# guenthermi/postgres-word2vec

Measured on AMD Instinct MI355X. Metric: batched IVFADC kNN queries/sec (k=5) + recall@5, 3Mx300d, higher is better.
Workload: dtype f32; 1 GPU; IVFADC batch (ivfadc_batch_search generalised to nprobe), 3000000x300d, C=1000, m=12, K=1024, nprobe=10, k=5, batch=1024 queries per GPU, replicated index, queries sharded by rank; N=3000000, d=300, C=1000, m=12, K=1024, nprobe=10, k=5, batch_per_gpu=1024, parallelism=dp1, world_size=1, backend=none (single GPU), batches_in_flight=4

## Files before the change

postgres-word2vec_amd/csrc/core.hip:

```cpp
#include "internal.h"

static thread_local char g_err[512] = "";

int fail(int code, const char* fmt, ...) {
  va_list ap;
  va_start(ap, fmt);
  vsnprintf(g_err, sizeof(g_err), fmt, ap);
  va_end(ap);
  return code;
}

extern "C" const char* freddy_gpu_last_error(void) { return g_err; }

#include "registry.h"

void backend_handles(int delta, int device) { freddy::registry::handles(delta, device); }
int backends_other(bool searching, int device) { return freddy::registry::others(searching, device); }
void backend_busy(int delta) { freddy::registry::busy(delta); }
void choose_hw_queues(int device) {
  static std::once_flag once;
  std::call_once(once, [device] {
    const char* policy = getenv("FREDDY_GPU_HWQ_POLICY");
    const bool alone = backends_other(false, device) == 0;
    const char* q = (policy && *policy && strcmp(policy, "registry") != 0) ? policy : (alone ? "6" : "2");
    setenv("GPU_MAX_HW_QUEUES", q, 0);
  });
}

int64_t env_int(const char* name, int64_t dflt) {
  const char* e = getenv(name);
  return (e && *e) ? (int64_t)strtoll(e, nullptr, 10) : dflt;
}
Tuning read_tuning() {
  Tuning t;
  t.fused = (int)env_int("FREDDY_GPU_FUSED", t.fused);
  t.scan_kernel = (int)env_int("FREDDY_GPU_FUSED_KERNEL", t.scan_kernel);
  t.reserve_cus = (int)env_int("FREDDY_GPU_RESERVE_CUS", 0);
  t.scan_share = (int)std::max<int64_t>(0, env_int("FREDDY_GPU_SCAN_SHARE", t.scan_share));
  t.pipeline_batch = (int)std::max<int64_t>(16, env_int("FREDDY_GPU_PIPELINE_BATCH", t.pipeline_batch));
  t.pipeline_lanes = (int)std::min<int64_t>(4, std::max<int64_t>(1, env_int("FREDDY_GPU_PIPELINE_LANES", t.pipeline_lanes)));
  t.pq_fused = (int)env_int("FREDDY_GPU_PQ_FUSED", t.pq_fused);
  t.one_launch = (int)env_int("FREDDY_GPU_ONE_LAUNCH", t.one_launch);
  t.coarse_approx = (int)env_int("FREDDY_GPU_COARSE_APPROX", 1);
  t.sparse_items = (int)env_int("FREDDY_GPU_SPARSE_ITEMS", t.sparse_items);
  t.exact_filter = (int)env_int("FREDDY_GPU_EXACT_FILTER", t.exact_filter);
  t.codes_u8 = (int)env_int("FREDDY_GPU_CODES_U8", t.codes_u8);
  t.running_bound = (int)env_int("FREDDY_GPU_RUNNING_BOUND", t.running_bound);
  t.lut_budget_mb = std::max<int64_t>(1, env_int("FREDDY_GPU_LUT_BUDGET_MB", t.lut_budget_mb));
  t.lane0_own = (int)env_int("FREDDY_GPU_LANE0_OWN", t.lane0_own);
  t.coarse_pieces = (int)env_int("FREDDY_GPU_COARSE_PIECES", t.coarse_pieces);
#ifdef FREDDY_LAB
  t.scan_prof = getenv("FREDDY_GPU_FUSED_PROF") != nullptr;
#endif
  return t;
}

Workspace* workspace_for(freddy_gpu_index* ix, hipStream_t s) {
  std::lock_guard<std::mutex> lock(ix->mu);
  Workspace* w = nullptr;
  for (Workspace& c : ix->ws)
    if (c.used && c.owner == s) { w = &c; break; }
  if (!w)
    for (Workspace& c : ix->ws)
      if (!c.used) { c.used = true; c.owner = s; w = &c; break; }
  if (!w) {
    w = &ix->ws[0];
    for (Workspace& c : ix->ws)
      if (c.last_use < w->last_use) w = &c;
    (void)hipDeviceSynchronize();
    w->owner = s;
  }
  w->last_use = ++ix->ws_clock;
  ix->last_ws = w;
  return w;
}

void free_index(freddy_gpu_index* ix) {
  if (!ix) return;
  if (ix->registered) { ix->registered = false; backend_handles(-1, ix->device); }
  for (freddy_gpu_index* r : ix->replicas) free_index(r);
  ix->replicas.clear();
  (void)hipSetDevice(ix->device);
  (void)hipDeviceSynchronize();
// ... 122 lines not shown
  if (!ix || !name) return fail(FREDDY_E_ARG, "NULL argument");
  if (!ix->replicas.empty()) {
    std::vector<freddy_gpu_index*> reps;
    reps.swap(ix->replicas);
    int rc = freddy_gpu_set_option(ix, name, value);
    reps.swap(ix->replicas);
    if (rc) return rc;
    for (freddy_gpu_index* r : ix->replicas)
      if ((rc = freddy_gpu_set_option(r, name, value))) { ix->poisoned = true; return rc; }
    return FREDDY_OK;
  }
  Tuning& t = ix->tune;
  const std::string n(name);
  if (n == "fused") t.fused = (int)value;
  else if (n == "fused_kernel") t.scan_kernel = (int)value;
  else if (n == "reserve_cus") t.reserve_cus = (int)value;
  else if (n == "scan_share") t.scan_share = (int)std::max<int64_t>(0, value);
  else if (n == "join_host_traversal") ix->join.host_traversal = value != 0;
  else if (n == "join_libm_margin_ppm") ix->join.libm_margin = (float)value * 1e-6f;
  else if (n == "sparse_items") t.sparse_items = std::max(-16, std::min(16, (int)value));
  else if (n == "pipeline_batch") t.pipeline_batch = (int)std::max<int64_t>(16, value);
  else if (n == "pipeline_lanes") t.pipeline_lanes = (int)std::min<int64_t>(FREDDY_LANES, std::max<int64_t>(1, value));
  else if (n == "pq_fused") t.pq_fused = (int)value;
  else if (n == "one_launch") t.one_launch = (int)value;
  else if (n == "coarse_approx") t.coarse_approx = (int)value;
  else if (n == "check_brackets") t.check_brackets = (int)value;
  else if (n == "lut_budget_mb") t.lut_budget_mb = std::max<int64_t>(1, value);
  else if (n == "exact_filter") t.exact_filter = (int)value;
  else if (n == "exact_join_tile") t.exact_join_tile = (int)value;
  else if (n == "analogy_pass") t.analogy_pass = (int)std::max<int64_t>(0, std::min<int64_t>(value, 1 << 30));
  else if (n == "codes_u8") t.codes_u8 = (int)value;
  else if (n == "running_bound") t.running_bound = (int)value;
  else if (n == "coarse_pieces") t.coarse_pieces = (int)value;
#ifdef FREDDY_LAB
  else if (n == "fused_prof") t.scan_prof = (int)value;
  else if (n == "scan_fence") t.scan_fence = (int)value;
#endif
  else return fail(FREDDY_E_ARG, "unknown option '%s'", name);
  return FREDDY_OK;
}

int check_search_args(const freddy_gpu_index* ix, int kind, const void* q, int Q, int k, const void* oi,
                             const void* od) {
  if (!ix) return fail(FREDDY_E_ARG, "NULL index");
  if (ix->kind != kind) return fail(FREDDY_E_KIND, "index handle has the wrong kind for this call");
  if (ix->poisoned) return fail(FREDDY_E_HIP, "this handle's devices hold different tables (an append / codebook update failed part-way): unpin it and pin again");
  if (Q < 0 || k <= 0) return fail(FREDDY_E_ARG, "Q must be >= 0 and k > 0");
  if (Q > 0 && (!q || !oi || !od)) return fail(FREDDY_E_ARG, "NULL buffer");
  if (k > 4096) return fail(FREDDY_E_LIMIT, "k=%d exceeds this build's limit of 4096", k);
  return 0;
}

extern "C" int freddy_gpu_host_alloc(void** out, size_t bytes) {
  choose_hw_queues(-1);
  if (!out) return fail(FREDDY_E_ARG, "NULL argument");
  *out = nullptr;
  if (hipHostMalloc(out, bytes ? bytes : 1, hipHostMallocDefault) != hipSuccess) { *out = nullptr; return fail(FREDDY_E_NOMEM, "pinned host allocation of %zu bytes failed", bytes); }
  return FREDDY_OK;
}
extern "C" int freddy_gpu_host_free(void* p) {
  if (p) HIP_TRY(hipHostFree(p));
  return FREDDY_OK;
}

extern "C" int freddy_gpu_replica_count(const freddy_gpu_index_t* ix) { return ix ? 1 + (int)ix->replicas.size() : 0; }
extern "C" int freddy_gpu_abi_version(void) { return FREDDY_GPU_ABI_VERSION; }
// ... 1 lines not shown
```

postgres-word2vec_amd/csrc/fused5.h:

```cpp
#pragma once
#include <hip/hip_runtime.h>
#include <stdint.h>

#include "refine.h"
#include "coarse.h"
#include "scan_tail5.h"

namespace freddy {

static constexpr int SCAN5_G = 16;

__host__ __device__ __forceinline__ constexpr int filt5_bias(int p, int m) { return FILT5_VMAX + (p < 32768 - FILT5_VMAX * m ? 1 : 0); }
__device__ __forceinline__ uint32_t lane_byte4() {
  uint32_t x;
  asm volatile("v_mbcnt_lo_u32_b32 %0, -1, 0\n\tv_mbcnt_hi_u32_b32 %0, -1, %0\n\tv_lshlrev_b32 %0, 2, %0" : "=v"(x));
  return x;
}
typedef short s2v __attribute__((ext_vector_type(2)));
__device__ __forceinline__ uint32_t pk_add_i16(uint32_t x, uint32_t y) {
  return __builtin_bit_cast(uint32_t, __builtin_bit_cast(s2v, x) + __builtin_bit_cast(s2v, y));
}

template <int S, int QT>
__device__ __forceinline__ void query_codebook5_body(const float* __restrict__ queries, const float* __restrict__ cbT,
// ... 91 lines not shown
                                                             const float* __restrict__ cmax, float* __restrict__ qn,
                                                             float* __restrict__ qscale, uint32_t* __restrict__ qc,
                                                             int Q, int d, int m, int K, uint32_t* __restrict__ qc8) {
  __shared__ __attribute__((aligned(16))) unsigned char smem[query_codebook5_lds<S, QT>()];
  query_codebook5_body<S, QT>(queries, cbT, cmax, qn, qscale, qc, Q, d, m, K, blockIdx.x, blockIdx.y, smem, qc8);
}

struct CoarseTableArgs {
  const float* queries;
  const float* coarseF; const float* cn2; float* dist; float* qn2; int Q, Cpad, d, dp; ZeroArgs z; int coarse_gx, coarse_gy;
  const float* cbT; const float* cmax; float* qn; float* qscale; uint32_t* qc; int m, K;
  float* tmin; int C;
  const ch8v* coarseH; int ec;
  uint32_t* qc8;
};
template <int S, int QT, bool H16 = false>
__global__ __launch_bounds__(256) void coarse_table5_kernel(CoarseTableArgs a) {
  extern __shared__ __attribute__((aligned(16))) unsigned char smem[];
  const int n_coarse = a.coarse_gx * a.coarse_gy;
  const int b = blockIdx.x;
  if (b < n_coarse) {
    if constexpr (H16)
      coarse_approx16_body(a.queries, a.coarseH, a.ec, a.cn2, a.dist, a.qn2, a.Q, a.Cpad, a.d, a.z, b % a.coarse_gx, b / a.coarse_gx,
                           a.coarse_gx, a.coarse_gy, smem, a.tmin, a.C);
    else
    coarse_approx_body(a.queries, a.coarseF, a.cn2, a.dist, a.qn2, a.Q, a.Cpad, a.d, a.dp, a.z, b % a.coarse_gx, b / a.coarse_gx,
                       a.coarse_gx, a.coarse_gy, smem, a.tmin, a.C);
  } else {
    const int t = b - n_coarse;
    query_codebook5_body<S, QT>(a.queries, a.cbT, a.cmax, a.qn, a.qscale, a.qc, a.Q, a.d, a.m, a.K, t % a.m, t / a.m, smem, a.qc8);
  }
}

template <int M>
__global__ __launch_bounds__(256) void entry_record5_kernel(RecordArgs a) {
  const int lane = threadIdx.x & 63;
  const int e = blockIdx.x * 4 + (threadIdx.x >> 6);
  if (e >= a.n_groups[0]) return;
  const int cell = a.group_cell[e], first = a.group_first[e], gc = a.group_cnt[e];
  const int cnt = gc & 0xff, chunk = gc >> 8;
  int32_t* rec = a.records + (size_t)e * REC_DW;
  if (lane == 0) {
    const int b0 = a.blk_off[cell] + chunk * FUSED_UNIT_BLOCKS;
    int nb = a.blk_off[cell + 1] - b0;
    if (nb > FUSED_UNIT_BLOCKS) nb = FUSED_UNIT_BLOCKS;
    int rows = a.list_off[cell + 1] - a.list_off[cell] - chunk * (FUSED_UNIT_BLOCKS * 64);
    if (rows > FUSED_UNIT_BLOCKS * 64) rows = FUSED_UNIT_BLOCKS * 64;
    rec[0] = cell; rec[1] = cnt; rec[2] = chunk; rec[3] = b0; rec[4] = nb; rec[5] = rows;
  }
  if (lane < 16) {
    const int it = lane < cnt ? a.sorted_item[first + lane] : -1;
    const int q = a.item_query[it >= 0 ? it : a.sorted_item[first]];
    const float sc = a.qscale[q];
    ItemBounds ib = item_bounds(0.0f, 0.0f, a.sentinel);
    if (it >= 0) ib = item_bounds(a.item_dist[it], filter_width5<M>(a.qn + (size_t)q * M, a.pmax, sc), a.sentinel);
    rec[8 + lane] = it;
    rec[24 + lane] = q;
    rec[40 + lane] = (int32_t)__float_as_uint(ib.off);
    rec[56 + lane] = (int32_t)__float_as_uint(ib.e);
    rec[72 + lane] = (int32_t)__float_as_uint(ib.shift);
    rec[88 + lane] = (int32_t)ib.lo_bits;
    rec[104 + lane] = (int32_t)ib.hi_bits;
    rec[128 + lane] = (int32_t)__float_as_uint((it >= 0 && sc < 1e30f) ? sc : 0.0f);
    const float A = it >= 0 ? a.item_dist[it] : -1.0f;
    const bool fin = it >= 0 && ib.e < 1e30f && A >= 0.0f && A < 1e30f;
    rec[144 + lane] = (int32_t)__float_as_uint(fin ? A * (1.0f + 2e-5f) : __uint_as_float(0x7f800000u));
    rec[160 + lane] = (int32_t)__float_as_uint(fin ? A * (1.0f - 2e-5f) : 0.0f);
  }
}

template <int M, bool FULLK, bool CAND, bool PROF = false, bool U8 = false>
__global__ __launch_bounds__(SPEC2_T) void ivf_filter5_kernel(FilterArgs a) {
  static_assert(!(U8 && FULLK), "one byte per code: K <= 256");
  constexpr int G = SCAN5_G, RMAX = FUSED_RMAX, NG = SPEC2_NG;
  constexpr int NP = M / 2;
  constexpr int ROWB = G * 2;
  constexpr int HROWB = 16;
  static_assert(M == 12 && G == 16 && SPEC2_NB == 8, "layout");
  typedef uint32_t u2 __attribute__((ext_vector_type(2)));
  typedef uint32_t u4 __attribute__((ext_vector_type(4)));
  extern __shared__ __attribute__((aligned(16))) unsigned char smem[];
  unsigned char* slab = smem;
  uint32_t* colmin = reinterpret_cast<uint32_t*>(smem + a.desc_offset);
  uint32_t* thr_s = colmin + 16 * 64;
  int32_t* dsc = reinterpret_cast<int32_t*>(smem + a.desc_offset + 4096 + 64);
  int32_t* gidq = dsc + 2 * REC_DW;
  float* rt_s = reinterpret_cast<float*>(gidq + 4);

  const int tid = threadIdx.x, lane = tid & 63;
  const int wave = __builtin_amdgcn_readfirstlane(tid >> 6);
  const bool builder = wave < SPEC2_NB;
  const int K = FULLK ? 1024 : a.K;
  const uint32_t HALFB = (uint32_t)K * HROWB;
  const uint32_t POSB = 2u * HALFB;
  const uint32_t BUFB = 2u * POSB;
  const int n_work = a.n_groups[0];

  int cur = 0, ei = 0;
  if (tid == 0) { gidq[0] = (int)blockIdx.x; gidq[1] = (int)gridDim.x + atomicAdd(a.work_counter, 1); }
  if (tid < REC_DW) dsc[tid] = a.records[(size_t)blockIdx.x * REC_DW + tid];
  for (int i = tid; i < 16 * 64; i += SPEC2_T) colmin[i] = 0xffffffffu;
// ... 283 lines not shown
```

postgres-word2vec_amd/csrc/internal.h:

```cpp
#pragma once
#include "../../include/freddy_gpu.h"

#include <hip/hip_runtime.h>

#include <algorithm>
#include <atomic>
#include <thread>
#include <cmath>
#include <cstdarg>
#include <cstdio>
#include <cstdlib>
#include <cstring>
#include <limits>
#include <chrono>
#include <map>
#include <mutex>
#include <string>
#include <type_traits>
#include <vector>

#include "join_index.h"
#include "pinned.h"

using namespace freddy;

int fail(int code, const char* fmt, ...) __attribute__((format(printf, 2, 3)));

#define HIP_TRY(expr)                                                                       \
  do {                                                                                      \
    hipError_t e_ = (expr);                                                                 \
    if (e_ != hipSuccess)                                                                   \
      return fail(FREDDY_E_HIP, "%s failed: %s (%s:%d)", #expr, hipGetErrorString(e_),      \
                  __FILE__, __LINE__);                                                      \
  } while (0)

enum { KIND_PQ = 1, KIND_IVF = 2, KIND_IVPQ = 3, KIND_VEC = 4 };

struct Tuning {
  int scan_share = 0;
  int reserve_cus = 0;
  int pipeline_batch = 2048;
  int pipeline_lanes = 4;
  int lane0_own = 0;
  int coarse_pieces = 1;
  int64_t lut_budget_mb = 8192;
  int fused = -1;
  int scan_kernel = 5;
  int coarse_approx = 1;
  int one_launch = 1;
  int pq_fused = -1;
  int sparse_items = 2;
  int running_bound = 1;
  int codes_u8 = 1;
  int exact_filter = -1;
  int exact_join_tile = 0;
  int analogy_pass = 0;
  int check_brackets = 0;
#ifdef FREDDY_LAB
  int scan_prof = 0;
  int scan_fence = 0;
#endif
};
int64_t env_int(const char* name, int64_t dflt);
int backends_other(bool searching, int device);
void backend_handles(int delta, int device);
void backend_busy(int delta);
void choose_hw_queues(int device);
struct BackendBusy { BackendBusy() { backend_busy(1); } ~BackendBusy() { backend_busy(-1); } };
static inline int scan_share_now(int option, bool host_call, int device) { return option > 0 ? option : (host_call && backends_other(true, device) > 0 ? 2 : 1); }
Tuning read_tuning();

struct DevBuf {
  void* p = nullptr;
  size_t cap = 0;
  int ensure(size_t bytes) {
    if (bytes <= cap) return 0;
    if (p) (void)hipFree(p);
    p = nullptr;
    cap = 0;
    size_t want = bytes + bytes / 8 + 256;
    if (hipMalloc(&p, want) != hipSuccess) { p = nullptr; return -1; }
    cap = want;
    return 0;
  }
  void release() { if (p) (void)hipFree(p); p = nullptr; cap = 0; }
  template <class T> T* as() const { return reinterpret_cast<T*>(p); }
};

struct Workspace {
  bool used = false;
// ... 3 lines not shown
      w_part, w_cand, w_found, w_act0, w_act1, w_cnt, w_out_ids, w_out_dist, w_sub_rows,
      w_sub_packed, w_sub_pos, w_sub_blk, w_cellcnt, w_sorted, w_groups, w_surv, w_surv_cnt, w_prof, w_qc, w_qn, w_records, w_qn2, w_item_dist, w_tmin, w_one, w_oneb, w_bigsel, w_floor;
  uint64_t one_shape = 0;
  uint32_t one_epoch = 0;
  bool one_pending = false;
  void release() {
    DevBuf* bufs[] = {&w_q, &w_distT, &w_used, &w_item_cell, &w_item_query, &w_rows, &w_resid, &w_lut, &w_part,
                      &w_cand, &w_found, &w_act0, &w_act1, &w_cnt, &w_out_ids, &w_out_dist, &w_sub_rows, &w_sub_packed,
                      &w_sub_pos, &w_sub_blk, &w_cellcnt, &w_sorted, &w_groups, &w_surv, &w_surv_cnt, &w_prof, &w_qc,
                      &w_qn, &w_records, &w_qn2, &w_item_dist, &w_tmin, &w_one, &w_oneb, &w_bigsel, &w_floor};
    for (DevBuf* b : bufs) b->release();
    used = false;
    owner = nullptr;
  }
};
static constexpr int FREDDY_MAX_WS = 12;

struct IvfRun {
  freddy_gpu_index* ix;
  Workspace* ws;
  hipStream_t s;
  int share;
  const float* d_q;
  int Q, k, W, L, found_rule, upi;
  float sentinel, cell_limit;
  int32_t *d_out_ids, *d_status;
  float* d_out_dist;
  bool fused;
  int scan_kernel;
  bool tiled;
  bool zeroed;
  bool approx;
  bool records_ready;
  int merge_slices;
  int n_active, round;
  const int32_t* active;
  int32_t* next;
  bool first() const { return round == 0; }
};

struct LaneSlot {
  hipEvent_t done = nullptr;
  PinnedBuf h_in;
  PinnedBuf h_out;
  DevBuf d_q, d_ids, d_dist;
  bool busy = false;
  int q0 = 0, n = 0;
};
struct Lane {
  hipStream_t stream = nullptr;
  LaneSlot slot[2];
};
static constexpr int FREDDY_LANES = 4;

struct ProfRec {
  int64_t launches = 0;
  double ms = 0.0;
  std::vector<std::pair<hipEvent_t, hipEvent_t>> open;
};

struct freddy_gpu_index {
  int kind = 0;
  int device = 0;
  Tuning tune;
  hipStream_t stream = nullptr;
  int d = 0, m = 0, K = 0, C = 0, S = 0, M2 = 0;
// ... 191 lines not shown
```

postgres-word2vec_amd/csrc/ivfadc.hip:

```cpp
#include "internal.h"

#include <functional>

#include "kernels.h"
#include "scan_common.h"
#include "fused3.h"
#include "fused5.h"
#include "fused8.h"
#include "one.h"
#include "sparse5.h"
#include "coarse.h"
#include "multi.h"
#include "io_kernels.h"
#include "bigk.h"

int pick_V(int L) {
  if (L <= 64) return 1;
  if (L <= 128) return 2;
  if (L <= 256) return 4;
  if (L <= 512) return 8;
  if (L <= 1024) return 16;
  return 0;
}

// ... 85 lines not shown
  HIP_TRY(hipGetLastError());
  return 0;
}


static bool scan_whole_slab(const freddy_gpu_index* ix) { return ix->packed8 && ix->tune.codes_u8 == 1 && ix->K <= 256 && ix->m == 12; }
static bool ivf_coarse_by_pieces(const IvfRun& r) { return r.approx && r.fused && r.scan_kernel == 5; }
static int ivf_coarse(IvfRun& r, int q_lo = 0, int q_n = -1) {
  Workspace* ws = r.ws;
  freddy_gpu_index* ix = r.ix;
  hipStream_t s = r.s;
  const int Q = r.Q, d = ix->d, C = ix->C, m = ix->m, K = ix->K, Cpad = ix->Cpad;
  if (q_n < 0) { q_lo = 0; q_n = Q; }
  if ((q_lo != 0 || q_n != Q) && !ivf_coarse_by_pieces(r)) return fail(FREDDY_E_ARG, "internal: this path launches its coarse kernel once");
  const int used_words = (C + 31) / 32;
  const size_t items = (size_t)Q * r.W;
  const bool small_zero = !r.tiled && d <= 1024;
  if (!r.tiled && !small_zero) {
    HIP_TRY(hipMemsetAsync(ws->w_used.p, 0, sizeof(uint32_t) * (size_t)Q * used_words, s));
    HIP_TRY(hipMemsetAsync(ws->w_cnt.p, 0, sizeof(int32_t) * 8, s));
  }
  ZeroArgs za;
  za.p[0] = ws->w_used.as<uint32_t>(); za.n[0] = Q * used_words;
  za.p[1] = ws->w_cnt.as<uint32_t>(); za.n[1] = 8;
  za.p[2] = r.fused ? ws->w_cellcnt.as<uint32_t>() : nullptr; za.n[2] = r.fused ? C * 2 : 0;
  za.p[3] = ws->w_cand.as<uint32_t>(); za.n[3] = 2 * Q;
  za.p[4] = r.fused ? ws->w_surv_cnt.as<uint32_t>() : nullptr; za.n[4] = r.fused ? (int)(items * r.upi * FUSED_NW) : 0;

  float* tile_min = nullptr;
  if (r.approx && Cpad > COARSE_MAX_CPAD) {
    if (ws->w_tmin.ensure(sizeof(float) * (size_t)Q * (Cpad / 128))) return fail(FREDDY_E_NOMEM, "workspace allocation failed");
    tile_min = ws->w_tmin.as<float>();
  }
  auto launch_coarse = [&]() -> int {
    timed_launch(ix, s, "coarse_dist", [&] {
      if (r.approx && ix->coarseH)
        hipLaunchKernelGGL(coarse_approx16_kernel, dim3(Cpad / 128, (Q + COARSE_TQ - 1) / COARSE_TQ), dim3(256), coarse_approx16_lds(d), s, r.d_q,
                           (const ch8v*)ix->coarseH, ix->coarse_ec, ix->cn2, ws->w_distT.as<float>(), ws->w_qn2.as<float>(), Q, Cpad, d, za, tile_min, C);
      else if (r.approx)
        hipLaunchKernelGGL(coarse_approx_kernel, dim3(Cpad / 128, (Q + COARSE_TQ - 1) / COARSE_TQ), dim3(256),
                           (size_t)(COARSE_TQ * (ix->dp + 4) + 128) * sizeof(float), s, r.d_q, ix->coarseP, ix->cn2,
                           ws->w_distT.as<float>(), ws->w_qn2.as<float>(), Q, Cpad, d, ix->dp, za, tile_min, C);
      else if (r.tiled)
        hipLaunchKernelGGL((coarse_tile_kernel<2, 16>), dim3(Cpad / 32, (Q + 63) / 64), dim3(256), 0, s, r.d_q, ix->coarseT,
                           ws->w_distT.as<float>(), Q, Cpad, d, za);
      else if (small_zero)
        hipLaunchKernelGGL((coarse_small_kernel<50>), dim3(Cpad / 64, Q), dim3(64), 0, s, r.d_q, ix->coarseT, ws->w_distT.as<float>(), Q, Cpad, d, za);
      else
        hipLaunchKernelGGL((coarse_dist_kernel<16>), dim3(Cpad / WG, (Q + 15) / 16), dim3(WG), (size_t)d * 16 * sizeof(float), s, r.d_q,
                           ix->coarseT, ws->w_distT.as<float>(), Q, Cpad, d);
    });
    HIP_TRY(hipGetLastError());
    return 0;
  };
  if (r.approx && r.fused && r.scan_kernel == 5) {
    CoarseTableArgs ct;
    ct.queries = r.d_q + (size_t)q_lo * d; ct.coarseF = ix->coarseP; ct.cn2 = ix->cn2; ct.dist = ws->w_distT.as<float>() + (size_t)q_lo * Cpad;
    ct.qn2 = ws->w_qn2.as<float>() + q_lo;
    ct.Q = q_n; ct.Cpad = Cpad; ct.d = d; ct.dp = ix->dp; ct.z = za; ct.coarse_gx = Cpad / 128; ct.coarse_gy = (q_n + COARSE_TQ - 1) / COARSE_TQ;
    ct.cbT = ix->cbF; ct.cmax = ix->cmaxp; ct.qn = ws->w_qn.as<float>() + (size_t)q_lo * m; ct.qscale = ws->w_qn.as<float>() + (size_t)Q * m + q_lo;
    ct.qc = ws->w_qc.as<uint32_t>() + (size_t)q_lo * m * 512; ct.m = m; ct.K = K; ct.tmin = tile_min ? tile_min + (size_t)q_lo * (Cpad / 128) : nullptr; ct.C = C;
    ct.coarseH = (const ch8v*)ix->coarseH; ct.ec = ix->coarse_ec;
    ct.qc8 = scan_whole_slab(ix) ? ws->w_qc.as<uint32_t>() + (size_t)Q * m * 512 + (size_t)q_lo * m * 128 : nullptr;
    const size_t lds = std::max<size_t>(ix->coarseH ? coarse_approx16_lds(d) : (size_t)(COARSE_TQ * (ix->dp + 4) + 128) * sizeof(float), (size_t)query_codebook5_lds<25, 16>());
    const unsigned grid = (unsigned)(ct.coarse_gx * ct.coarse_gy + m * ((q_n + 15) / 16));
    timed_launch(ix, s, "coarse_table", [&] {
      if (ix->coarseH) hipLaunchKernelGGL((coarse_table5_kernel<25, 16, true>), dim3(grid), dim3(256), lds, s, ct);
      else hipLaunchKernelGGL((coarse_table5_kernel<25, 16>), dim3(grid), dim3(256), lds, s, ct);
    });
    HIP_TRY(hipGetLastError());
    return 0;
  }
  if (r.fused && r.scan_kernel == 5) {
    timed_launch(ix, s, "query_codebook", [&] {
      hipLaunchKernelGGL((query_codebook5_kernel<25, 16>), dim3(m, (Q + 15) / 16), dim3(256), 0, s, r.d_q, ix->cbF, ix->cmaxp,
                         ws->w_qn.as<float>(), ws->w_qn.as<float>() + (size_t)Q * m, ws->w_qc.as<uint32_t>(), Q, d, m, K,
                         scan_whole_slab(ix) ? ws->w_qc.as<uint32_t>() + (size_t)Q * m * 512 : nullptr);
    });
    HIP_TRY(hipGetLastError());
  }
  return launch_coarse();
}

static int ivf_plan(IvfRun& r, PlanArgs& pa) {
  Workspace* ws = r.ws;
  freddy_gpu_index* ix = r.ix;
  hipStream_t s = r.s;
  const int C = ix->C, W = r.W;
  pa.dist = ws->w_distT.as<float>(); pa.active = r.active; pa.list_off = ix->list_off;
  pa.used = ws->w_used.as<uint32_t>();
  pa.item_cell = ws->w_item_cell.as<int32_t>(); pa.item_query = ws->w_item_query.as<int32_t>();
  pa.item_dist = ws->w_item_dist.as<float>();
  pa.round_rows = ws->w_rows.as<int32_t>();
  pa.n_active = r.n_active; pa.Cpad = ix->Cpad; pa.C = C; pa.W = W; pa.used_words = (C + 31) / 32;
  pa.cell_count = r.fused ? ws->w_cellcnt.as<int32_t>() : nullptr;
  pa.cell_items = r.fused ? ws->w_sorted.as<int32_t>() : nullptr; pa.cell_cap = r.n_active;
  pa.cell_limit = r.cell_limit;
  const int n_items = r.n_active * W;
  if (r.fused && !(r.zeroed && r.first())) {
    HIP_TRY(hipMemsetAsync(ws->w_cellcnt.p, 0, sizeof(int32_t) * (size_t)C * 2, s));
    HIP_TRY(hipMemsetAsync(ws->w_surv_cnt.p, 0, sizeof(int32_t) * (size_t)n_items * r.upi * FUSED_NW, s));
  }
  const int PV = pick_V(2 * W);
  const size_t plan_lds = (size_t)(64 + 64 * PV) * sizeof(u64) + (size_t)W * 8;
  if (r.approx) {
    Plan2Args g;
    g.p = pa; g.queries = r.d_q; g.coarse = ix->coarse; g.qn2 = ws->w_qn2.as<float>(); g.item_dist = pa.item_dist;
    g.violations = ix->viol; g.cmax = ix->cmax; g.d = ix->d; g.refine_all = (ix->tune.check_brackets & 2) ? 1 : 0; g.prof = nullptr;
    g.tmin = (r.first() && ix->Cpad > COARSE_MAX_CPAD && ws->w_tmin.p) ? ws->w_tmin.as<float>() : nullptr;
    timed_launch(ix, s, "probe_plan", [&] {
      if (ix->Cpad <= COARSE_MAX_CPAD && r.share > 1) hipLaunchKernelGGL((probe_plan2_kernel<0, false, 1>), dim3(r.n_active), dim3(64), 0, s, g);
      else if (ix->Cpad <= COARSE_MAX_CPAD) hipLaunchKernelGGL((probe_plan2_kernel<0, false>), dim3(r.n_active), dim3(64 * PLAN2_NW), 0, s, g);
      else hipLaunchKernelGGL((probe_plan2_kernel<0, true>), dim3(r.n_active), dim3(64 * PLAN2_NW), 0, s, g);
    });
// ... 48 lines not shown
}

#ifdef FREDDY_LAB
static int scan_prof_print(freddy_gpu_index* ix, hipStream_t s, const long long* prof, unsigned n_persist) {
  std::vector<long long> h(8 * (size_t)n_persist);
  HIP_TRY(hipStreamSynchronize(s));
  HIP_TRY(hipMemcpy(h.data(), prof, sizeof(long long) * h.size(), hipMemcpyDeviceToHost));
  double sum[8] = {0}; long long mx_end = 0, mn_end = -1; double ent = 0;
  for (unsigned b = 0; b < n_persist; ++b) {
    for (int i = 0; i < 6; ++i) sum[i] += (double)h[b * 8 + i];
    ent += (double)h[b * 8 + 7];
    mx_end = std::max(mx_end, h[b * 8 + 6]);
    mn_end = mn_end < 0 ? h[b * 8 + 6] : std::min(mn_end, h[b * 8 + 6]);
  }
  fprintf(stderr, "[scan prof] wgs=%u entries=%.0f  builder cycles/entry: builds=%.0f barrier-wait=%.0f tail=%.0f | gatherer wave 0 (fused5.h): main=%.0f colmin=%.0f S2=%.0f | workgroups ran dry over %.1f us\n",
          n_persist, ent, sum[0] / ent, sum[1] / ent, sum[3] / ent, sum[2] / ent, sum[4] / ent, sum[5] / ent, (mx_end - mn_end) / 100.0);
  (void)ix;
  return 0;
}
#endif

int ivf_scan_filter(IvfRun& r, const PlanArgs& pa, const WorkTable& wt) {
  Workspace* ws = r.ws;
  freddy_gpu_index* ix = r.ix;
  hipStream_t s = r.s;
  const int Q = r.Q, m = ix->m, K = ix->K;
  if (!r.records_ready && ws->w_records.ensure(sizeof(int32_t) * REC_DW * wt.max_groups)) return fail(FREDDY_E_NOMEM, "workspace allocation failed");
  RecordArgs ra;
  ra.group_cell = wt.group_cell; ra.group_first = wt.group_first; ra.group_cnt = wt.group_cnt; ra.n_groups = wt.n_groups;
  ra.sorted_item = ws->w_sorted.as<int32_t>(); ra.item_query = pa.item_query; ra.blk_off = ix->blk_off; ra.list_off = ix->list_off;
  ra.item_dist = pa.item_dist; ra.qn = ws->w_qn.as<float>(); ra.qscale = ws->w_qn.as<float>() + (size_t)Q * m; ra.pmax = ix->pmax;
  ra.records = ws->w_records.as<int32_t>(); ra.sentinel = r.sentinel;
  if (!r.records_ready) {
    timed_launch(ix, s, "entry_records", [&] {
      hipLaunchKernelGGL((entry_record5_kernel<12>), dim3((unsigned)((wt.max_groups + 3) / 4)), dim3(256), 0, s, ra);
    });
    HIP_TRY(hipGetLastError());
  }
  FilterArgs fl;
  fl.qc = ws->w_qc.as<uint32_t>(); fl.qc8 = ws->w_qc.as<uint32_t>() + (size_t)Q * m * 512; fl.rterm = ix->rterm; fl.records = ws->w_records.as<int32_t>(); fl.n_groups = wt.n_groups;
  fl.work_counter = wt.work_counter; fl.packed = ix->packed; fl.surv = ws->w_surv.as<u64>(); fl.surv_count = ws->w_surv_cnt.as<int32_t>();
  fl.cand_count = (r.found_rule == 1) ? ws->w_cand.as<int32_t>() : nullptr;
  fl.K = K; fl.L = r.L; fl.upi = r.upi; fl.sentinel = r.sentinel; fl.keep_all = (ix->tune.check_brackets & 1) ? 1 : 0; fl.fence = 0;
#ifdef FREDDY_LAB
  fl.fence = (uint32_t)ix->tune.scan_fence;
#endif
  fl.tau_run = (ix->tune.running_bound && !r.records_ready) ? ws->w_cand.as<uint32_t>() + Q : nullptr;
  if (int rc = scan_prof_buffer(ix, ws, &fl.prof)) return rc;
  const bool u8 = ix->packed8 && ix->tune.codes_u8 != 0 && K <= 256;
  const bool whole = u8 && scan_whole_slab(ix);
  const size_t desc_off = whole ? (size_t)scan8_slab_bytes(12) : (size_t)4 * SCAN5_G * 2 * K;
  const size_t flds = desc_off + 4096 + 64 + (2 * REC_DW + 4) * sizeof(int32_t) + 4096 * sizeof(float);
  fl.desc_offset = (uint32_t)desc_off;
  const int scan_cus = std::max(ix->n_cus / std::max(1, r.share), std::min(ix->n_cus, 32)) - ix->tune.reserve_cus;
  const unsigned n_persist = (unsigned)std::min<size_t>(wt.max_groups, (size_t)std::max(1, scan_cus));
  fl.packed8 = u8 ? ix->packed8 : nullptr;
  timed_launch(ix, s, "ivf_filter", [&] {
    if (whole) {
#ifdef FREDDY_LAB
      if (fl.prof && !fl.cand_count) hipLaunchKernelGGL((ivf_filter8_kernel<12, false, true>), dim3(n_persist), dim3(SPEC2_T), flds, s, fl);
      else
#endif
      if (fl.cand_count) hipLaunchKernelGGL((ivf_filter8_kernel<12, true>), dim3(n_persist), dim3(SPEC2_T), flds, s, fl);
      else hipLaunchKernelGGL((ivf_filter8_kernel<12, false>), dim3(n_persist), dim3(SPEC2_T), flds, s, fl);
    } else if (u8) {
      if (fl.cand_count) hipLaunchKernelGGL((ivf_filter5_kernel<12, false, true, false, true>), dim3(n_persist), dim3(SPEC2_T), flds, s, fl);
      else hipLaunchKernelGGL((ivf_filter5_kernel<12, false, false, false, true>), dim3(n_persist), dim3(SPEC2_T), flds, s, fl);
    } else if (fl.cand_count) {
      if (K == 1024) hipLaunchKernelGGL((ivf_filter5_kernel<12, true, true>), dim3(n_persist), dim3(SPEC2_T), flds, s, fl);
      else hipLaunchKernelGGL((ivf_filter5_kernel<12, false, true>), dim3(n_persist), dim3(SPEC2_T), flds, s, fl);
// ... 190 lines not shown
  if (int rc = ivf_plan(r, pa)) return rc;
  if (r.fused) {
    WorkTable wt;
    if (int rc = ivf_work_table(r, wt)) return rc;
    return (r.scan_kernel == 5) ? ivf_scan_filter(r, pa, wt) : (r.scan_kernel == 2) ? ivf_scan_multi(r, pa, wt) : ivf_scan_exact(r, pa, wt);
  }
  return ivf_scan_generic(r, pa);
}

static int ivfadc_begin(freddy_gpu_index* ix, hipStream_t s, int share, const float* d_q, int Q, int k, int W,
                        float sentinel, int found_rule, int32_t* d_out_ids, float* d_out_dist,
                        int32_t* d_status, IvfRun& r, const std::function<int(int, int)>* stage = nullptr, bool by_pieces = false) {
  Workspace* ws = workspace_for(ix, s);
  const int C = ix->C, m = ix->m, K = ix->K;
  if (2 * W > 1024) return fail(FREDDY_E_LIMIT, "W=%d exceeds this build's limit of 512 probes per round", W);
  r.ix = ix; r.ws = ws; r.s = s; r.d_q = d_q; r.Q = Q; r.k = k; r.W = W; r.L = std::min(2 * k, 64 * 16);
  r.sentinel = sentinel; r.d_out_ids = d_out_ids; r.d_out_dist = d_out_dist; r.d_status = d_status;
  r.share = std::max(1, share);
  r.found_rule = found_rule == FREDDY_FOUND_ROWS ? 0 : 1;
  r.cell_limit = found_rule == FREDDY_FOUND_BATCH_UDF ? 1000.0f : 100.0f;
  const size_t items = (size_t)Q * W;
  r.upi = std::max(1, (ix->max_list_blocks + FUSED_UNIT_BLOCKS - 1) / FUSED_UNIT_BLOCKS);
  r.fused = ix->tune.fused != 0 && m == 12 && ix->S == 25 && K <= 1024 && ix->cbP && r.L <= 64 && r.upi <= 8 &&
            (ix->tune.fused == 1 || items >= 256);
  r.scan_kernel = (ix->tune.scan_kernel == 3 || !ix->rterm) ? 3 : 5;
  if (!r.fused) {
    const bool special = m == 12 && ix->S == 25 && K <= 1024 && ix->cbP;
    r.fused = ix->tune.fused != 0 && !special && multi_lds_bytes(m, K) <= (size_t)150 * 1024 && r.L <= 64 && r.upi <= 32 &&
              (ix->tune.fused == 1 || items >= 256);
    if (r.fused) r.scan_kernel = 2;
  }
  r.tiled = Q >= 32;
  r.zeroed = r.tiled || ix->d <= 1024;
  r.records_ready = false; r.merge_slices = 0;
  r.approx = ix->tune.coarse_approx != 0 && r.tiled && ix->Cpad <= COARSE_STREAM_MAX_CPAD && 2 * W <= 64 && ix->d <= 300 && ix->d % 4 == 0 && ix->coarseP;
  const int Cpad = ix->Cpad, used_words = (C + 31) / 32;
  if (ws->w_distT.ensure(sizeof(float) * (size_t)Q * Cpad) ||
      ws->w_used.ensure(sizeof(uint32_t) * (size_t)Q * used_words) ||
      ws->w_item_cell.ensure(sizeof(int32_t) * items) || ws->w_item_query.ensure(sizeof(int32_t) * items) ||
      ws->w_rows.ensure(sizeof(int32_t) * Q) || ws->w_cand.ensure(sizeof(int32_t) * 2 * Q) ||
      ws->w_qn2.ensure(sizeof(float) * Q) || ws->w_item_dist.ensure(sizeof(float) * items) ||
      ws->w_found.ensure(sizeof(int32_t) * Q) || ws->w_act0.ensure(sizeof(int32_t) * Q) ||
      ws->w_act1.ensure(sizeof(int32_t) * Q) || ws->w_cnt.ensure(sizeof(int32_t) * 8))
    return fail(FREDDY_E_NOMEM, "workspace allocation failed (Q=%d, W=%d)", Q, W);
  if (r.fused) {
    if (ws->w_cellcnt.ensure(sizeof(int32_t) * (size_t)C * 3) || ws->w_sorted.ensure(sizeof(int32_t) * (size_t)C * Q) ||
        ws->w_groups.ensure(sizeof(int32_t) * 3 * ((items / MULTI_G + (size_t)C + 1) * r.upi + items * r.upi)) ||
        ws->w_surv.ensure(sizeof(u64) * items * r.upi * FUSED_NW * FUSED_RMAX * 64) ||
        ws->w_surv_cnt.ensure(sizeof(int32_t) * items * r.upi * FUSED_NW))
      return fail(FREDDY_E_NOMEM, "workspace allocation failed (Q=%d, W=%d)", Q, W);
    if (r.scan_kernel == 2 && ws->w_lut.ensure(sizeof(float) * items * (size_t)m * K))
      return fail(FREDDY_E_NOMEM, "workspace allocation failed (Q=%d, W=%d)", Q, W);
    if (r.scan_kernel == 5 &&
        (ws->w_qc.ensure(sizeof(uint32_t) * (size_t)Q * m * 640) || ws->w_qn.ensure(sizeof(float) * (size_t)Q * m * 2)))
      return fail(FREDDY_E_NOMEM, "workspace allocation failed (Q=%d, W=%d)", Q, W);
  } else {
    const size_t nchunk_big = (size_t)std::max(1, (ix->max_list_blocks + 255) / 256), nchunk_small = (size_t)std::max(1, (ix->max_list_blocks + 31) / 32);
    const size_t parts = std::max(items * nchunk_big, std::min<size_t>(items, 64) * nchunk_small);
    if (ws->w_resid.ensure(sizeof(float) * items * (size_t)ix->d) || ws->w_lut.ensure(sizeof(float) * items * (size_t)m * K) ||
        ws->w_part.ensure(sizeof(u64) * parts * r.L))
      return fail(FREDDY_E_NOMEM, "workspace allocation failed (Q=%d, W=%d)", Q, W);
  }

  const int pieces = (stage && by_pieces && ix->tune.coarse_pieces && ivf_coarse_by_pieces(r) && Q >= 512) ? 4 : 1;
  const int per = ((Q + pieces - 1) / pieces + 31) & ~31;
  for (int q_lo = 0; q_lo < Q; q_lo += (pieces > 1 ? per : Q)) {
    const int q_n = pieces > 1 ? std::min(per, Q - q_lo) : Q;
// ... 361 lines not shown
```

postgres-word2vec_amd/csrc/pq.hip:

```cpp
#include "internal.h"

#include "kernels.h"
#include "scan_common.h"
#include "fused5.h"
#include "one.h"
#include "io_kernels.h"
#include "assign.h"

__global__ __launch_bounds__(256) void pq_shadow_meta_kernel(const int32_t* __restrict__ pos, const int32_t* __restrict__ ids,
                                                            int64_t n_blocks, int64_t n_rows, int lists, int32_t* __restrict__ list_off,
                                                            int32_t* __restrict__ blk_off, int32_t* __restrict__ blk_cell,
                                                            int32_t* __restrict__ pos_ids) {
  const int64_t i = (int64_t)blockIdx.x * 256 + threadIdx.x;
  if (i <= lists) {
    const int64_t r = i * (FUSED_UNIT_BLOCKS * 64), b = i * FUSED_UNIT_BLOCKS;
    list_off[i] = (int32_t)(r < n_rows ? r : n_rows);
    blk_off[i] = (int32_t)(b < n_blocks ? b : n_blocks);
  }
  if (i < n_blocks) blk_cell[i] = (int32_t)(i / FUSED_UNIT_BLOCKS);
  if (i < n_blocks * 64) { const int32_t r = pos[i]; pos_ids[i] = r >= 0 ? ids[r] : -1; }
}

static bool pq_fused_shape(const freddy_gpu_index* ix) {
  return ix->kind == KIND_PQ && ix->cbR && ix->m == 12 && ix->S == 25 && ix->K <= FUSED_T * FUSED_E && ix->n_blocks > 0 && ix->N > 0;
// ... 136 lines not shown
  fx->coarse = fx->v_coarse.as<float>(); fx->list_off = fx->v_list_off.as<int32_t>(); fx->blk_off = fx->v_blk_off.as<int32_t>();
  fx->blk_cell = fx->v_blk_cell.as<int32_t>(); fx->pos = fx->v_pos.as<int32_t>(); fx->rterm = fx->v_rterm.as<float>();
  HIP_TRY(hipMemsetAsync(fx->coarse, 0, sizeof(float) * (size_t)lists * ix->d, s));
  hipLaunchKernelGGL(pq_shadow_meta_kernel, dim3((unsigned)((slots + 255) / 256)), dim3(256), 0, s, pos, ix->ids, n_blocks, n_rows, lists,
                     fx->list_off, fx->blk_off, fx->blk_cell, fx->pos);
  hipLaunchKernelGGL(row_term_kernel, dim3((unsigned)((slots + 255) / 256)), dim3(256), 0, s, fx->packed, fx->blk_cell, fx->coarse, fx->cbR,
                     fx->rterm, (int64_t)slots, fx->M2, fx->d, fx->m, fx->K, fx->S);
  HIP_TRY(hipGetLastError());
  return 0;
}

int pq_shadow_build(freddy_gpu_index* ix) {
  if (ix->pq_shadow) return 0;
  if (int rc = pq_view_refresh(ix, &ix->pq_shadow, ix->stream, ix->packed, ix->pos, ix->n_blocks, ix->N)) {
    if (ix->pq_shadow) { free_index(ix->pq_shadow); ix->pq_shadow = nullptr; }
    return rc;
  }
  HIP_TRY(hipStreamSynchronize(ix->stream));
  return 0;
}


static int pq_fused_chunk(freddy_gpu_index* ix, freddy_gpu_index* fx, hipStream_t s, const float* d_q, int Q, int k, float sentinel,
                          int32_t* d_out_ids, float* d_out_dist) {
  fx->tune = ix->tune;
  Workspace* ws = workspace_for(fx, s);
  const int lists = fx->C, m = fx->m, K = fx->K;
  const int SL = (lists >= 32 && Q <= 256 && (size_t)lists * FUSED_NW > 256) ? 4 : 0;
  const int W = SL ? ((lists + SL - 1) / SL) * SL : lists;
  IvfRun r;
  r.ix = fx; r.ws = ws; r.s = s; r.d_q = d_q; r.Q = Q; r.k = k; r.W = W; r.L = 2 * k;
  r.sentinel = sentinel; r.cell_limit = 0.0f; r.d_out_ids = d_out_ids; r.d_out_dist = d_out_dist; r.d_status = nullptr;
  r.found_rule = 0; r.upi = 1; r.fused = true; r.scan_kernel = 5; r.tiled = false; r.zeroed = false; r.approx = false;
  r.records_ready = true; r.merge_slices = SL;
  r.n_active = Q; r.round = 0; r.active = nullptr;
  r.share = scan_share_now(ix->tune.scan_share, false, ix->device);
  const size_t items = (size_t)Q * W;
  const size_t n_entries = (size_t)((Q + SCAN5_G - 1) / SCAN5_G) * lists;
  if (ws->w_item_cell.ensure(sizeof(int32_t) * items) || ws->w_item_query.ensure(sizeof(int32_t) * items) ||
      ws->w_item_dist.ensure(sizeof(float) * items) || ws->w_rows.ensure(sizeof(int32_t) * Q) || ws->w_cand.ensure(sizeof(int32_t) * 2 * Q) ||
      ws->w_found.ensure(sizeof(int32_t) * Q) || ws->w_act0.ensure(sizeof(int32_t) * Q) || ws->w_act1.ensure(sizeof(int32_t) * Q) ||
      ws->w_cnt.ensure(sizeof(int32_t) * 8) || ws->w_records.ensure(sizeof(int32_t) * REC_DW * n_entries) ||
      ws->w_surv.ensure(sizeof(u64) * items * r.upi * FUSED_NW * FUSED_RMAX * 64) ||
      ws->w_surv_cnt.ensure(sizeof(int32_t) * items * r.upi * FUSED_NW) ||
      ws->w_qc.ensure(sizeof(uint32_t) * (size_t)Q * m * 640) || ws->w_qn.ensure(sizeof(float) * (size_t)Q * m * 2))
    return fail(FREDDY_E_NOMEM, "workspace allocation failed (Q=%d over %d pseudo-lists)", Q, lists);
  r.next = ws->w_act0.as<int32_t>();
  PlanArgs pa;
  memset(&pa, 0, sizeof(pa));
  pa.item_cell = ws->w_item_cell.as<int32_t>(); pa.item_query = ws->w_item_query.as<int32_t>(); pa.item_dist = ws->w_item_dist.as<float>();
  pa.round_rows = ws->w_rows.as<int32_t>(); pa.n_active = Q; pa.C = lists; pa.W = W;
  WorkTable wt;
  wt.max_groups = n_entries; wt.group_cell = wt.group_first = wt.group_cnt = nullptr;
  wt.n_groups = ws->w_cnt.as<int32_t>() + 1; wt.work_counter = ws->w_cnt.as<int32_t>() + 2;
  wt.sp_cap = 0; wt.sp_cell = wt.sp_first = wt.sp_chunk = nullptr; wt.sp_counter = ws->w_cnt.as<int32_t>() + 3; wt.n_sparse = ws->w_cnt.as<int32_t>() + 4;
  PqFrontArgs fa;
  fa.queries = d_q; fa.Q = Q; fa.d = fx->d; fa.lists = lists; fa.W = W; fa.n_rows = fx->N; fa.blk_off = fx->blk_off; fa.list_off = fx->list_off;
  fa.cbT = fx->cbF; fa.cmax = fx->cmaxp; fa.pmax = fx->pmax; fa.qn = ws->w_qn.as<float>(); fa.qscale = ws->w_qn.as<float>() + (size_t)Q * m;
  fa.qc = ws->w_qc.as<uint32_t>(); fa.m = m; fa.K = K; fa.sentinel = sentinel;
  fa.qc8 = (fx->packed8 && fx->tune.codes_u8 == 1 && K <= 256 && m == 12) ? ws->w_qc.as<uint32_t>() + (size_t)Q * m * 512 : nullptr; fa.item_cell = pa.item_cell; fa.item_query = pa.item_query;
  fa.item_dist = pa.item_dist; fa.round_rows = pa.round_rows; fa.records = ws->w_records.as<int32_t>(); fa.n_groups = wt.n_groups;
  fa.z.p[0] = ws->w_cnt.as<uint32_t>(); fa.z.n[0] = 1;
  fa.z.p[1] = ws->w_cnt.as<uint32_t>() + 2; fa.z.n[1] = 6;
  fa.z.p[2] = ws->w_cand.as<uint32_t>() + Q; fa.z.n[2] = Q;
  fa.z.p[3] = ws->w_surv_cnt.as<uint32_t>(); fa.z.n[3] = (int)(items * r.upi * FUSED_NW);
  fa.z.p[4] = nullptr; fa.z.n[4] = 0;
  const size_t front_lds = std::max<size_t>((size_t)query_codebook5_lds<25, 16>(), (size_t)(1024 + 16 + 2) * sizeof(float));
// ... 320 lines not shown
```

Before: 11.26 million queries/s.

## Defer query codebook table build into the entry-records launch

By default the coarse step now launches only the coarse-distance kernel. The query-codebook LUT build is merged into one combined kernel with the entry-record construction. The record blocks work out per-subspace query norms and the scale themselves instead of reading them from the table output, so the two parts can run side by side in one grid. This cuts a launch and lets the coarse kernel run without the LUT blocks, but the record blocks repeat norm arithmetic, and the numerical bounds must match those the table kernel computes. An inspect_records debug option that copies the records out is also added.

Result: slower. 11.09 million queries/s (-1.6%).

```diff
diff --git a/postgres-word2vec_amd/csrc/core.hip b/postgres-word2vec_amd/csrc/core.hip
--- a/postgres-word2vec_amd/csrc/core.hip
+++ b/postgres-word2vec_amd/csrc/core.hip
@@ -49,6 +49,7 @@
   t.lut_budget_mb = std::max<int64_t>(1, env_int("FREDDY_GPU_LUT_BUDGET_MB", t.lut_budget_mb));
   t.lane0_own = (int)env_int("FREDDY_GPU_LANE0_OWN", t.lane0_own);
   t.coarse_pieces = (int)env_int("FREDDY_GPU_COARSE_PIECES", t.coarse_pieces);
+  t.table_launch = (int)env_int("FREDDY_GPU_TABLE_LAUNCH", t.table_launch);
 #ifdef FREDDY_LAB
   t.scan_prof = getenv("FREDDY_GPU_FUSED_PROF") != nullptr;
 #endif
@@ -237,6 +238,9 @@
   else if (n == "codes_u8") t.codes_u8 = (int)value;
   else if (n == "running_bound") t.running_bound = (int)value;
   else if (n == "coarse_pieces") t.coarse_pieces = (int)value;
+  else if (n == "table_launch") t.table_launch = (int)value;
+  else if (n == "inspect_records") t.inspect_records = value;
+  else if (n == "inspect_records_dwords") t.inspect_dwords = std::max<int64_t>(0, value);
 #ifdef FREDDY_LAB
   else if (n == "fused_prof") t.scan_prof = (int)value;
   else if (n == "scan_fence") t.scan_fence = (int)value;
diff --git a/postgres-word2vec_amd/csrc/fused5.h b/postgres-word2vec_amd/csrc/fused5.h
--- a/postgres-word2vec_amd/csrc/fused5.h
+++ b/postgres-word2vec_amd/csrc/fused5.h
@@ -147,10 +147,10 @@
   }
 }
 
-template <int M>
-__global__ __launch_bounds__(256) void entry_record5_kernel(RecordArgs a) {
+template <int M, int S, bool DERIVE>
+__device__ __forceinline__ void entry_record5_body(const RecordArgs& a, int e, const float* __restrict__ queries,
+                                                   const float* __restrict__ cmax, int d) {
   const int lane = threadIdx.x & 63;
-  const int e = blockIdx.x * 4 + (threadIdx.x >> 6);
   if (e >= a.n_groups[0]) return;
   const int cell = a.group_cell[e], first = a.group_first[e], gc = a.group_cnt[e];
   const int cnt = gc & 0xff, chunk = gc >> 8;
@@ -163,12 +163,36 @@
     if (rows > FUSED_UNIT_BLOCKS * 64) rows = FUSED_UNIT_BLOCKS * 64;
     rec[0] = cell; rec[1] = cnt; rec[2] = chunk; rec[3] = b0; rec[4] = nb; rec[5] = rows;
   }
+  float qnl[M];
+  float scl = 0.0f;
+  if constexpr (DERIVE) {
+    static_assert(M % 4 == 0, "a quarter of the positions per 16-lane group");
+    constexpr int PER = M / 4;
+    const int g = lane & 15, part = lane >> 4;
+    const int itg = g < cnt ? a.sorted_item[first + g] : -1;
+    const int qg = a.item_query[itg >= 0 ? itg : a.sorted_item[first]];
+    float nr[PER];
+#pragma unroll
+    for (int u = 0; u < PER; ++u) {
+      const float* qp = queries + (size_t)qg * d + (part * PER + u) * S;
+      float n2 = 0.0f;
+      for (int j = 0; j < S; ++j) { const float v = qp[j]; n2 = __builtin_fmaf(v, v, n2); }
+      nr[u] = __builtin_sqrtf(n2) * (1.0f + 1e-5f);
+    }
+    float best = 0.0f;
+#pragma unroll
+    for (int p = 0; p < M; ++p) {
+      qnl[p] = __shfl(nr[p % PER], g + 16 * (p / PER), 64);
+      best = fmaxf(best, 2.0f * qnl[p] * cmax[p]);
+    }
+    scl = best * (1.0f / (float)FILT5_VMAX) * (1.0f + 1e-6f);
+  }
   if (lane < 16) {
     const int it = lane < cnt ? a.sorted_item[first + lane] : -1;
     const int q = a.item_query[it >= 0 ? it : a.sorted_item[first]];
-    const float sc = a.qscale[q];
+    const float sc = DERIVE ? scl : a.qscale[q];
     ItemBounds ib = item_bounds(0.0f, 0.0f, a.sentinel);
-    if (it >= 0) ib = item_bounds(a.item_dist[it], filter_width5<M>(a.qn + (size_t)q * M, a.pmax, sc), a.sentinel);
+    if (it >= 0) ib = item_bounds(a.item_dist[it], filter_width5<M>(DERIVE ? qnl : a.qn + (size_t)q * M, a.pmax, sc), a.sentinel);
     rec[8 + lane] = it;
     rec[24 + lane] = q;
     rec[40 + lane] = (int32_t)__float_as_uint(ib.off);
@@ -182,6 +206,24 @@
     rec[144 + lane] = (int32_t)__float_as_uint(fin ? A * (1.0f + 2e-5f) : __uint_as_float(0x7f800000u));
     rec[160 + lane] = (int32_t)__float_as_uint(fin ? A * (1.0f - 2e-5f) : 0.0f);
   }
+}
+template <int M>
+__global__ __launch_bounds__(256) void entry_record5_kernel(RecordArgs a) {
+  entry_record5_body<M, 25, false>(a, blockIdx.x * 4 + (threadIdx.x >> 6), nullptr, nullptr, 0);
+}
+
+struct RecordTableArgs {
+  RecordArgs rec;
+  const float* queries; const float* cbT; const float* cmax; float* qn; float* qscale; uint32_t* qc;
+  uint32_t* qc8;
+  int Q, d, m, K, n_table;
+};
+template <int M, int S, int QT>
+__global__ __launch_bounds__(256) void record_table5_kernel(RecordTableArgs a) {
+  extern __shared__ __attribute__((aligned(16))) unsigned char smem[];
+  const int b = blockIdx.x;
+  if (b < a.n_table) query_codebook5_body<S, QT>(a.queries, a.cbT, a.cmax, a.qn, a.qscale, a.qc, a.Q, a.d, a.m, a.K, b % a.m, b / a.m, smem, a.qc8);
+  else entry_record5_body<M, S, true>(a.rec, (b - a.n_table) * 4 + (int)(threadIdx.x >> 6), a.queries, a.cmax, a.d);
 }
 
 template <int M, bool FULLK, bool CAND, bool PROF = false, bool U8 = false>
diff --git a/postgres-word2vec_amd/csrc/internal.h b/postgres-word2vec_amd/csrc/internal.h
--- a/postgres-word2vec_amd/csrc/internal.h
+++ b/postgres-word2vec_amd/csrc/internal.h
@@ -55,7 +55,10 @@
   int exact_filter = -1;
   int exact_join_tile = 0;
   int analogy_pass = 0;
+  int table_launch = 1;
   int check_brackets = 0;
+  int64_t inspect_records = 0;
+  int64_t inspect_dwords = 0;
 #ifdef FREDDY_LAB
   int scan_prof = 0;
   int scan_fence = 0;
@@ -125,6 +128,7 @@
   bool zeroed;
   bool approx;
   bool records_ready;
+  bool table_pending;
   int merge_slices;
   int n_active, round;
   const int32_t* active;
diff --git a/postgres-word2vec_amd/csrc/ivfadc.hip b/postgres-word2vec_amd/csrc/ivfadc.hip
--- a/postgres-word2vec_amd/csrc/ivfadc.hip
+++ b/postgres-word2vec_amd/csrc/ivfadc.hip
@@ -141,15 +141,19 @@
     if (ws->w_tmin.ensure(sizeof(float) * (size_t)Q * (Cpad / 128))) return fail(FREDDY_E_NOMEM, "workspace allocation failed");
     tile_min = ws->w_tmin.as<float>();
   }
-  auto launch_coarse = [&]() -> int {
-    timed_launch(ix, s, "coarse_dist", [&] {
+  auto launch_coarse = [&](const char* name) -> int {
+    const float* pq = r.d_q + (size_t)q_lo * d;
+    float* pdist = ws->w_distT.as<float>() + (size_t)q_lo * Cpad;
+    float* pqn2 = ws->w_qn2.as<float>() + q_lo;
+    float* ptmin = tile_min ? tile_min + (size_t)q_lo * (Cpad / 128) : nullptr;
+    timed_launch(ix, s, name, [&] {
       if (r.approx && ix->coarseH)
-        hipLaunchKernelGGL(coarse_approx16_kernel, dim3(Cpad / 128, (Q + COARSE_TQ - 1) / COARSE_TQ), dim3(256), coarse_approx16_lds(d), s, r.d_q,
-                           (const ch8v*)ix->coarseH, ix->coarse_ec, ix->cn2, ws->w_distT.as<float>(), ws->w_qn2.as<float>(), Q, Cpad, d, za, tile_min, C);
+        hipLaunchKernelGGL(coarse_approx16_kernel, dim3(Cpad / 128, (q_n + COARSE_TQ - 1) / COARSE_TQ), dim3(256), coarse_approx16_lds(d), s, pq,
+                           (const ch8v*)ix->coarseH, ix->coarse_ec, ix->cn2, pdist, pqn2, q_n, Cpad, d, za, ptmin, C);
       else if (r.approx)
-        hipLaunchKernelGGL(coarse_approx_kernel, dim3(Cpad / 128, (Q + COARSE_TQ - 1) / COARSE_TQ), dim3(256),
-                           (size_t)(COARSE_TQ * (ix->dp + 4) + 128) * sizeof(float), s, r.d_q, ix->coarseP, ix->cn2,
-                           ws->w_distT.as<float>(), ws->w_qn2.as<float>(), Q, Cpad, d, ix->dp, za, tile_min, C);
+        hipLaunchKernelGGL(coarse_approx_kernel, dim3(Cpad / 128, (q_n + COARSE_TQ - 1) / COARSE_TQ), dim3(256),
+                           (size_t)(COARSE_TQ * (ix->dp + 4) + 128) * sizeof(float), s, pq, ix->coarseP, ix->cn2,
+                           pdist, pqn2, q_n, Cpad, d, ix->dp, za, ptmin, C);
       else if (r.tiled)
         hipLaunchKernelGGL((coarse_tile_kernel<2, 16>), dim3(Cpad / 32, (Q + 63) / 64), dim3(256), 0, s, r.d_q, ix->coarseT,
                            ws->w_distT.as<float>(), Q, Cpad, d, za);
@@ -162,7 +166,10 @@
     HIP_TRY(hipGetLastError());
     return 0;
   };
-  if (r.approx && r.fused && r.scan_kernel == 5) {
+  const bool table5 = r.fused && r.scan_kernel == 5;
+  r.table_pending = table5 && ix->tune.table_launch != 0;
+  if (r.table_pending) return launch_coarse(r.approx ? "coarse_table" : "coarse_dist");
+  if (r.approx && table5) {
     CoarseTableArgs ct;
     ct.queries = r.d_q + (size_t)q_lo * d; ct.coarseF = ix->coarseP; ct.cn2 = ix->cn2; ct.dist = ws->w_distT.as<float>() + (size_t)q_lo * Cpad;
     ct.qn2 = ws->w_qn2.as<float>() + q_lo;
@@ -180,7 +187,7 @@
     HIP_TRY(hipGetLastError());
     return 0;
   }
-  if (r.fused && r.scan_kernel == 5) {
+  if (table5) {
     timed_launch(ix, s, "query_codebook", [&] {
       hipLaunchKernelGGL((query_codebook5_kernel<25, 16>), dim3(m, (Q + 15) / 16), dim3(256), 0, s, r.d_q, ix->cbF, ix->cmaxp,
                          ws->w_qn.as<float>(), ws->w_qn.as<float>() + (size_t)Q * m, ws->w_qc.as<uint32_t>(), Q, d, m, K,
@@ -188,7 +195,7 @@
     });
     HIP_TRY(hipGetLastError());
   }
-  return launch_coarse();
+  return launch_coarse("coarse_dist");
 }
 
 static int ivf_plan(IvfRun& r, PlanArgs& pa) {
@@ -303,10 +310,30 @@
   ra.item_dist = pa.item_dist; ra.qn = ws->w_qn.as<float>(); ra.qscale = ws->w_qn.as<float>() + (size_t)Q * m; ra.pmax = ix->pmax;
   ra.records = ws->w_records.as<int32_t>(); ra.sentinel = r.sentinel;
   if (!r.records_ready) {
-    timed_launch(ix, s, "entry_records", [&] {
-      hipLaunchKernelGGL((entry_record5_kernel<12>), dim3((unsigned)((wt.max_groups + 3) / 4)), dim3(256), 0, s, ra);
-    });
+    const unsigned rec_grid = (unsigned)((wt.max_groups + 3) / 4);
+    if (r.table_pending) {
+      RecordTableArgs rt;
+      rt.rec = ra; rt.queries = r.d_q; rt.cbT = ix->cbF; rt.cmax = ix->cmaxp; rt.qn = ws->w_qn.as<float>(); rt.qscale = ws->w_qn.as<float>() + (size_t)Q * m;
+      rt.qc = ws->w_qc.as<uint32_t>(); rt.qc8 = scan_whole_slab(ix) ? ws->w_qc.as<uint32_t>() + (size_t)Q * m * 512 : nullptr;
+      rt.Q = Q; rt.d = ix->d; rt.m = m; rt.K = K; rt.n_table = m * ((Q + 15) / 16);
+      const size_t lds = (size_t)query_codebook5_lds<25, 16>();
+      timed_launch(ix, s, "entry_records", [&] {
+        hipLaunchKernelGGL((record_table5_kernel<12, 25, 16>), dim3((unsigned)rt.n_table + rec_grid), dim3(256), lds, s, rt);
+      });
+      r.table_pending = false;
+    } else {
+      timed_launch(ix, s, "entry_records", [&] { hipLaunchKernelGGL((entry_record5_kernel<12>), dim3(rec_grid), dim3(256), 0, s, ra); });
+    }
     HIP_TRY(hipGetLastError());
+    if (ix->tune.inspect_records && r.first()) {
+      const size_t head = 1 + (size_t)Q * m + Q, cap = (size_t)ix->tune.inspect_dwords;
+      if (cap < head) return fail(FREDDY_E_ARG, "inspect_records_dwords=%zu is less than the %zu dwords of the counts, norms and scales", cap, head);
+      int32_t* dst = reinterpret_cast<int32_t*>((uintptr_t)ix->tune.inspect_records);
+      const size_t n_rec = std::min((size_t)REC_DW * wt.max_groups, cap - head);
+      HIP_TRY(hipMemcpyAsync(dst, wt.n_groups, 4, hipMemcpyDeviceToDevice, s));
+      HIP_TRY(hipMemcpyAsync(dst + 1, ws->w_qn.p, 4 * (head - 1), hipMemcpyDeviceToDevice, s));
+      if (n_rec) HIP_TRY(hipMemcpyAsync(dst + head, ws->w_records.p, 4 * n_rec, hipMemcpyDeviceToDevice, s));
+    }
   }
   FilterArgs fl;
   fl.qc = ws->w_qc.as<uint32_t>(); fl.qc8 = ws->w_qc.as<uint32_t>() + (size_t)Q * m * 512; fl.rterm = ix->rterm; fl.records = ws->w_records.as<int32_t>(); fl.n_groups = wt.n_groups;
@@ -563,7 +590,7 @@
   }
   r.tiled = Q >= 32;
   r.zeroed = r.tiled || ix->d <= 1024;
-  r.records_ready = false; r.merge_slices = 0;
+  r.records_ready = false; r.table_pending = false; r.merge_slices = 0;
   r.approx = ix->tune.coarse_approx != 0 && r.tiled && ix->Cpad <= COARSE_STREAM_MAX_CPAD && 2 * W <= 64 && ix->d <= 300 && ix->d % 4 == 0 && ix->coarseP;
   const int Cpad = ix->Cpad, used_words = (C + 31) / 32;
   if (ws->w_distT.ensure(sizeof(float) * (size_t)Q * Cpad) ||
diff --git a/postgres-word2vec_amd/csrc/pq.hip b/postgres-word2vec_amd/csrc/pq.hip
--- a/postgres-word2vec_amd/csrc/pq.hip
+++ b/postgres-word2vec_amd/csrc/pq.hip
@@ -192,7 +192,7 @@
   r.ix = fx; r.ws = ws; r.s = s; r.d_q = d_q; r.Q = Q; r.k = k; r.W = W; r.L = 2 * k;
   r.sentinel = sentinel; r.cell_limit = 0.0f; r.d_out_ids = d_out_ids; r.d_out_dist = d_out_dist; r.d_status = nullptr;
   r.found_rule = 0; r.upi = 1; r.fused = true; r.scan_kernel = 5; r.tiled = false; r.zeroed = false; r.approx = false;
-  r.records_ready = true; r.merge_slices = SL;
+  r.records_ready = true; r.table_pending = false; r.merge_slices = SL;
   r.n_active = Q; r.round = 0; r.active = nullptr;
   r.share = scan_share_now(ix->tune.scan_share, false, ix->device);
   const size_t items = (size_t)Q * W;
```
